# Varkalandar/raysnail

Hardware: AMD Instinct MI355X
Metric: Msamples/s (whole node) + ms/frame, RTIOW-13.1 scene 800x500x64spp (higher is better)
Workload: dtype f64; 1 GPU; rtow_13_1 balls_scene(seed 7)+light, 800x500, 64 spp, depth 8; width=800, height=500, spp=64, depth=8, split=rows, lanes=default, frames_in_flight=default, samples_per_frame=25600000

## Files before the change

raysnail_amd/csrc/rs_host.cpp:

```cpp
#include <hip/hip_runtime.h>

#include <algorithm>
#include <atomic>
#include <chrono>
#include <functional>
#include <cmath>
#include <cstdio>
#include <cstdlib>
#include <cstring>
#include <memory>
#include <new>
#include <stdexcept>
#include <string>
#include <vector>

#include "../../include/raysnail_hip.h"
#include "rs_host_util.h"
#include "rs_internal.h"
#include "rs_layout.h"
#include "rs_cull.h"

using namespace rs;

namespace {

thread_local std::string g_last_error;

struct Box3 {
    double lo[3], hi[3];
};
Box3 box_union(const Box3& a, const Box3& b) {
    Box3 r;
    for (int i = 0; i < 3; ++i) { r.lo[i] = std::fmin(a.lo[i], b.lo[i]); r.hi[i] = std::fmax(a.hi[i], b.hi[i]); }
    return r;
}
Box3 box_empty() {
    Box3 r;
    for (int i = 0; i < 3; ++i) { r.lo[i] = INFINITY; r.hi[i] = -INFINITY; }
    return r;
}

struct HObj {
    int32_t kind = 0;
    int32_t mat = RS_NO_MATERIAL;
    double p[18] = {0};
    int32_t a = -1, b = -1;
    int32_t ax[3] = {0, 0, 0};
    std::vector<rs_transform> tfs;
};

struct HPerlin {
    rs_perlin_desc d;
    std::vector<double> values;
// ... 78 lines not shown
};

struct CandKey {
    DCamera dc{};
    uint32_t width = 0, height = 0, row_begin = 0, row_step = 0, n_pix = 0;
    uint64_t gen = 0;
    bool valid = false;
    bool same(const CandKey& o) const {
        return valid && o.valid && std::memcmp(&dc, &o.dc, sizeof(DCamera)) == 0 && width == o.width && height == o.height &&
               row_begin == o.row_begin && row_step == o.row_step && n_pix == o.n_pix && gen == o.gen;
    }
};

struct Slot {
    hipStream_t lane[kMaxLanes] = {nullptr};
    hipEvent_t fork_ev = nullptr, join_ev[kMaxLanes] = {nullptr};
    hipEvent_t free_ev = nullptr, entry_ev = nullptr;
    bool free_rec = false;
    double* d_rad = nullptr; size_t rad_cap = 0;
    double* d_acc = nullptr; size_t acc_cap = 0;
    unsigned long long* d_cnt = nullptr;
    uint8_t* d_mask = nullptr; size_t mask_cap = 0;
    float* d_out = nullptr; size_t out_cap = 0;
    float* d_feat = nullptr; size_t feat_cap = 0;
    void* d_wf = nullptr; size_t wf_cap = 0; uint32_t wf_lanes = 0; size_t wf_bytes = 0;
    QEnt** d_qptrs[kMaxLanes] = {nullptr};
    QEnt* qptr[kMaxLanes][kWfsClasses] = {{nullptr}};
    WfState lane_ws[kMaxLanes]{};
    uint32_t* d_counts = nullptr; size_t counts_cap = 0;
    size_t counts_clean = 0;
    hipStream_t acc_stream = nullptr;
    std::vector<hipEvent_t> bev;
    uint32_t* h_hist = nullptr; size_t hist_cap = 0, hist_words = 0; uint64_t hist_sig = 0;
    hipEvent_t hist_ev = nullptr; bool hist_pending = false;
    uint4* d_cand = nullptr; size_t cand_cap = 0;
    CandKey cand_key{};

    void quiesce() {
        for (uint32_t l = 0; l < kMaxLanes; ++l)
            if (lane[l]) HIP_OK(hipStreamSynchronize(lane[l]));
        if (acc_stream) HIP_OK(hipStreamSynchronize(acc_stream));
        if (free_rec) HIP_OK(hipEventSynchronize(free_ev));
    }
    void release() {
        for (uint32_t l = 0; l < kMaxLanes; ++l)
            if (lane[l]) (void)hipStreamSynchronize(lane[l]);
        if (acc_stream) (void)hipStreamSynchronize(acc_stream);
        if (free_rec) (void)hipEventSynchronize(free_ev);
        for (void* p : {(void*)d_rad, (void*)d_acc, (void*)d_cnt, (void*)d_mask, (void*)d_out, (void*)d_feat, d_wf, (void*)d_counts,
                        (void*)d_cand})
            if (p) (void)hipFree(p);
        for (uint32_t l = 0; l < kMaxLanes; ++l) {
            if (lane[l]) (void)hipStreamDestroy(lane[l]);
            if (join_ev[l]) (void)hipEventDestroy(join_ev[l]);
        }
        for (hipEvent_t e : {fork_ev, free_ev, entry_ev})
            if (e) (void)hipEventDestroy(e);
        for (hipEvent_t e : bev) (void)hipEventDestroy(e);
        if (acc_stream) (void)hipStreamDestroy(acc_stream);
        if (hist_ev) (void)hipEventDestroy(hist_ev);
        if (h_hist) (void)hipHostFree(h_hist);
    }
};

struct Replica {
    int device = 0;
    hipStream_t stream = nullptr;
    DScene ds{};
    std::vector<void*> dev;
    Slot slots[kMaxSlots];
    uint32_t next_slot = 0;
    int n_cu = 0, ext_bpc = 0, shade_bpc = 0;
    uint64_t mem_total = 0;
    int32_t* d_ovf = nullptr; size_t ovf_cap = 0;
    DScene* d_ds = nullptr;
    DScene uploaded{};
    std::vector<uint32_t> hist;
    uint64_t hist_sig = 0;
    std::vector<hipStream_t> pad_streams;

    void quiesce() {
        for (Slot& sl : slots) sl.quiesce();
        if (stream) HIP_OK(hipStreamSynchronize(stream));
    }
    SceneRef ref() {
        if (std::memcmp(&uploaded, &ds, sizeof(DScene)) != 0) {
            quiesce();
            HIP_OK(hipMemcpy(d_ds, &ds, sizeof(DScene), hipMemcpyHostToDevice));
            uploaded = ds;
        }
        return SceneRef{&ds, d_ds};
    }

    ~Replica() {
        int prev = -1;
        const bool switched = hipGetDevice(&prev) == hipSuccess && prev != device && hipSetDevice(device) == hipSuccess;
        for (Slot& sl : slots) sl.release();
        if (stream) (void)hipStreamSynchronize(stream);
        for (hipStream_t st : pad_streams) (void)hipStreamDestroy(st);
        for (void* p : dev) (void)hipFree(p);
        for (void* p : {(void*)d_ovf, (void*)d_ds})
            if (p) (void)hipFree(p);
        if (stream) (void)hipStreamDestroy(stream);
        if (switched) (void)hipSetDevice(prev);
    }
};

struct rs_scene {
    std::vector<rs_material_desc> mdesc;
    std::vector<HPerlin> perlins;
    std::vector<HImage> images;
    std::vector<HObj> objs;
    std::vector<uint32_t> world, lights;
    float bg_lo[3] = {0.3f, 0.4f, 0.5f}, bg_hi[3] = {0.7f, 0.89f, 1.0f};
    bool committed = false;
    bool spheres_only = false;
    int scene_mode = kSmGeneric;
    bool ref_order = false;
    HostScene hs;
    std::vector<std::unique_ptr<Replica>> reps;
    uint64_t max_items_per_batch = 32ull << 20;
    uint64_t pool_paths = 256ull << 20;
    uint32_t inject_div = 1;
    uint32_t finish_after = 16;
    uint32_t wf_lanes = 2;
    uint32_t stream_lanes = 1;
    uint32_t frames_in_flight = 3;
    bool ext_split = false;
    bool shade_split = true;
    bool dump_iters = false;
    uint32_t passes_stream = 0;
    uint32_t class_mask = (1u << kWfsClasses) - 1;
    int tree_depth = 0;
    int tree_arity = 0;
    int stack_need = 0;
    uint64_t commit_gen = 0;
    size_t n_nodes = 0;
    size_t n_leaf_entries = 0;
    double time0 = 0.0, time1 = 0.0;

    uint32_t add(HObj o) {
        if (committed) throw Error(RS_E_STATE, "scene already committed");
        objs.push_back(std::move(o));
        return (uint32_t)(objs.size() - 1);
    }
    void check_mat(int32_t m) const {
        if (m != RS_NO_MATERIAL && (m < 0 || (size_t)m >= mdesc.size())) throw Error(RS_E_INVALID, "unknown material id");
    }
    void check_handle(uint32_t h) const {
        if (h >= objs.size()) throw Error(RS_E_INVALID, "unknown object handle");
    }

    Box3 bbox(uint32_t h) { return bbox_t(h, time0, time1); }
    Box3 bbox_t(uint32_t h, double time0, double time1) {
        const HObj& o = objs[h];
        Box3 r;
        switch (o.kind) {
        case PK_SPHERE: {
            const double* c = o.p; const double rad = o.p[3]; const double* v = o.p + 5;
            Box3 s, e;
            if (v[0] == 0.0 && v[1] == 0.0 && v[2] == 0.0) {
                for (int i = 0; i < 3; ++i) { s.lo[i] = c[i] - rad; s.hi[i] = c[i] + rad; }
                return s;
// ... 855 lines not shown
    std::vector<double> tf64;
    std::vector<int32_t> ti32;
    for (const HPerlin& hp : s->perlins) {
        DPerlin x;
        std::memset(&x, 0, sizeof(x));
        x.point_count = (int32_t)hp.d.point_count; x.vector = hp.d.vector; x.smooth = hp.d.smooth; x.type = hp.d.type;
        x.depth = (int32_t)hp.d.depth; x.scale = hp.d.scale;
        x.voff = (int32_t)tf64.size(); x.poff = (int32_t)ti32.size();
        tf64.insert(tf64.end(), hp.values.begin(), hp.values.end());
        ti32.insert(ti32.end(), hp.perms.begin(), hp.perms.end());
        dper.push_back(x);
    }
    std::vector<DImage> dimg;
    std::vector<uint8_t> tu8;
    for (const HImage& hi : s->images) {
        DImage x; x.w = hi.w; x.h = hi.h; x.off = tu8.size();
        tu8.insert(tu8.end(), hi.rgb.begin(), hi.rgb.end());
        dimg.push_back(x);
    }
    stage(s, d.perlins, dper);
    stage(s, d.tex_f64, tf64);
    stage(s, d.tex_i32, ti32);
    stage(s, d.images, dimg);
    stage(s, d.tex_u8, tu8);
    d.uv = 0;
    for (const DMaterial& m : mats) if (m.tex_kind == RS_TEX_IMAGE) d.uv = 1;
    stage(s, d.lights, lights);
    d.n_lights = (int32_t)lights.size();
    d.root = root;
    d.default_mat = default_mat;
    d.ref_order = s->ref_order ? 1 : 0;
    for (int i = 0; i < 3; ++i) { d.bg_lo[i] = s->bg_lo[i]; d.bg_hi[i] = s->bg_hi[i]; }
    d.bg_lo[3] = d.bg_hi[3] = 1.0f;
    build_limg(s);
}

void commit(rs_scene* s, const int* devices, int n) {
    if (s->committed) throw Error(RS_E_STATE, "scene already committed");
    if (n < 0 || (n > 1 && !devices)) throw Error(RS_E_INVALID, "bad device list");
    build(s);
    int current = 0;
    if (n == 1 && !devices) {
        HIP_OK(hipGetDevice(&current));
        devices = &current;
    }
    int count = 0;
    if (n > 0) HIP_OK(hipGetDeviceCount(&count));
    for (int i = 0; i < n; ++i)
        if (devices[i] < 0 || devices[i] >= count) throw Error(RS_E_INVALID, "device ordinal out of range");
    int prev = 0;
    if (n > 0) HIP_OK(hipGetDevice(&prev));
    try {
        for (int i = 0; i < n; ++i) upload_replica(s, devices[i]);
        for (int i = 0; i < n; ++i)
            for (int j = 0; j < n; ++j) {
                if (devices[i] == devices[j]) continue;
                int can = 0;
                if (hipDeviceCanAccessPeer(&can, devices[i], devices[j]) == hipSuccess && can) {
                    (void)hipSetDevice(devices[i]);
                    (void)hipDeviceEnablePeerAccess(devices[j], 0);
                    (void)hipGetLastError();
                }
            }
    } catch (...) {
        s->reps.clear();
        (void)hipSetDevice(prev);
// ... 399 lines not shown
void accumulate_last(const Pending& P, const double* rad, uint32_t planes, bool first, const FinalParams& fp, float* out) {
    const size_t nz = P.counted ? 0 : P.n_counts;
    HIP_OK(launch_accumulate(rad, P.L->d_acc, P.n_pix, planes, first, 1, fp, out, P.L->d_counts, (uint32_t)nz, P.stream));
    P.L->counts_clean = nz;
}

struct PoolNeed { uint64_t cap; uint32_t lanes; size_t rad; };
template <class Plan, class Alloc>
void fit_pool(const rs_scene* s, const Replica& R, Slot& L, uint32_t want, uint64_t floor, Plan plan, Alloc alloc) {
    uint64_t pool = pool_limit(s, R, want);
    PoolNeed need = plan(pool);
    const uint64_t pool_min = std::min<uint64_t>(need.cap, floor);
    if (need.cap > L.wf_cap || need.lanes > L.wf_lanes || need.rad > L.rad_cap) {
        const uint64_t fp = std::max(pool_min, pool_limit_free(s, R, L, want, need.rad * sizeof(double)));
        if (fp < pool) need = plan(pool = fp);
    }
    while (!alloc(need)) {
        if (pool <= pool_min) throw Error(RS_E_NOMEM, "device memory exhausted: no room for the frame's path pool");
        need = plan(pool = std::max<uint64_t>(pool_min, pool / 2));
    }
}

void enqueue_empty(const FrameConsts& c, Pending& P) {
    Slot& L = *P.L;
    HIP_OK(hipMemsetAsync(L.d_acc, 0, (size_t)3 * P.n_pix * sizeof(double), L.lane[0]));
    join_to_end(L, P.stream);
    HIP_OK(launch_finalize(L.d_acc, c.d_out, c.fp, P.stream));
}

struct GridHist {
    uint64_t sig = 0;
    std::vector<size_t> hoff;
    size_t hwords = 0;
    bool hint = false;
};
GridHist hist_begin(Replica& R, Slot& L, const FrameSched& f, uint32_t n_pix, uint32_t N, uint32_t D, uint32_t n_frames) {
    GridHist h;
    h.sig = splitmix64_h(((uint64_t)n_pix << 32) ^ N) ^ splitmix64_h(((uint64_t)D << 40) ^ ((uint64_t)f.lanes << 32) ^ n_frames);
    for (const LaneSched& ln : f.lane) {
        h.sig = splitmix64_h(h.sig ^ ln.Q ^ (ln.T << 40) ^ (ln.total << 1) ^ (uint64_t)ln.finish);
        h.hoff.push_back(h.hwords);
        h.hwords += 2 * ln.T;
    }
    for (Slot& o : R.slots) {
        if (!o.hist_pending) continue;
        const hipError_t q = hipEventQuery(o.hist_ev);
        if (q == hipSuccess) {
            o.hist_pending = false;
            R.hist.assign(o.h_hist, o.h_hist + o.hist_words);
            R.hist_sig = o.hist_sig;
        } else {
            (void)hipGetLastError();
            if (q != hipErrorNotReady) HIP_OK(q);
        }
    }
#ifndef RS_NO_GRID_HINT
    h.hint = R.hist_sig == h.sig && R.hist.size() == h.hwords;
#endif
    if (L.hist_cap < h.hwords) {
        if (L.h_hist) { HIP_OK(hipEventSynchronize(L.hist_ev)); HIP_OK(hipHostFree(L.h_hist)); L.h_hist = nullptr; }
        HIP_OK(hipHostMalloc((void**)&L.h_hist, h.hwords * sizeof(uint32_t)));
        L.hist_cap = h.hwords;
        L.hist_pending = false;
    }
    if (!L.hist_ev) HIP_OK(hipEventCreateWithFlags(&L.hist_ev, hipEventDisableTiming));
    return h;
}
uint64_t hist_grid(const GridHist& h, const Replica& R, uint32_t l, uint64_t t, int word, uint64_t n_max, uint64_t more = 0) {
    if (!h.hint) return n_max;
    const uint64_t est = R.hist[h.hoff[l] + 2 * t + word];
    return std::min<uint64_t>(n_max, est + est / 4 + 64ull * kBlock + more);
}
void hist_end(const GridHist& h, Slot& L, const FrameSched& f, hipStream_t S) {
    for (uint32_t l = 0; l < f.lanes; ++l)
        HIP_OK(hipMemcpy2DAsync(L.h_hist + h.hoff[l], 2 * sizeof(uint32_t), L.d_counts + f.lane[l].cnt_off,
                                kWfsStride * sizeof(uint32_t), 2 * sizeof(uint32_t), f.lane[l].T,
                                hipMemcpyDeviceToHost, S));
    HIP_OK(hipEventRecord(L.hist_ev, S));
    L.hist_pending = true;
    L.hist_sig = h.sig;
    L.hist_words = h.hwords;
}

bool cam_cand_scene(const rs_scene* s, const DScene& d) {
    return cam_cand(s->scene_mode, kExtCamera) && d.moving == 0 && d.lsphs && d.root4 >= 0 && !d.ref_order &&
           s->objs.size() <= kCandMaxEntries && s->stack_need <= kCandStack;
}
const uint4* cam_cand_records(const rs_scene* s, const FrameConsts& c, Slot& L, hipStream_t L0) {
    const PathParams& pp = c.pp;
    if (!cam_cand_scene(s, *c.ds.host) || pp.n_pix_local == 0 || pp.n_pix_local > (0xFFFFFFFFu >> 4)) return nullptr;
    if (!cand_camera(c.dc.origin, c.dc.lb, c.dc.hf, c.dc.vf, c.dc.hu, c.dc.vu, c.dc.aperture, pp.width, pp.height).ok)
        return nullptr;
    CandKey key;
    key.dc = c.dc;
    key.width = pp.width; key.height = pp.height; key.row_begin = pp.row_begin; key.row_step = pp.row_step;
    key.n_pix = pp.n_pix_local;
    key.gen = s->commit_gen;
    key.valid = true;
    if (L.cand_key.same(key)) return L.d_cand;
    L.cand_key.valid = false;
    if (!try_ensure(L, L.d_cand, L.cand_cap, std::max<size_t>(pp.n_pix_local, (size_t)pp.width * pp.height))) return nullptr;
    HIP_OK(launch_cam_cand_build(c.ds, c.dc, pp, L.d_cand, L0));
    L.cand_key = key;
    return L.d_cand;
}

struct StreamFrame {
    const rs_scene* s; const FrameConsts& c; Pending& P; Slot& L;
    const uint4* cand = nullptr;
    FrameSched f;
    GridHist h;
    bool split, split_shade;
    std::vector<uint64_t> window;
    hipEvent_t done_ev(uint32_t k) const { return L.bev[2 * (size_t)k]; }
    hipEvent_t acc_ev(uint32_t k) const { return L.bev[2 * (size_t)k + 1]; }
    void iteration(uint32_t l, uint64_t t);
    void accumulate(uint32_t k);
};

void StreamFrame::iteration(uint32_t l, uint64_t t) {
    const bool timed = P.timed;
    const uint32_t D = P.depth;
    const int sm = s->scene_mode;
    const LaneSched& ln = f.lane[l];
    const hipStream_t cs = L.lane[l];
    WfState WS = L.lane_ws[l];
    WS.tagw = tag_in_ray(c.ds, c.dc);
    WS.counts = L.d_counts + ln.cnt_off;
    QEnt** qd = L.d_qptrs[l];
    const uint32_t n_new = ln.n_new(t);
    P.inj[l][t] = n_new;
    InjParams I = inj_params(f, ln, t);
    I.cand = cand;
    if (n_new) {
        const uint64_t m = t * ln.Q / f.B;
        for (uint64_t mm = m; mm <= m + 1 && mm < ln.batch.size(); ++mm) {
            const uint32_t kk = ln.batch[mm];
            if (ln.first_it(mm) == t && kk >= f.ring) HIP_OK(hipStreamWaitEvent(cs, acc_ev(kk - f.ring), 0));
        }
    }
    if (ln.finish && t + 1 == ln.T) {
        const uint32_t b = (uint32_t)std::min<uint64_t>(c.wide, (window[l] + kBlock - 1) / kBlock);
        if (timed) HIP_OK(hipEventRecord(P.kev[2 * P.ki], cs));
        HIP_OK(launch_wfs_finish(c.ds, WS, (uint32_t)t, D, L.d_rad, std::max<uint32_t>(1, b), sm, cs));
        if (timed) HIP_OK(hipEventRecord(P.kev[2 * P.ki + 1], cs));
        ++P.ki;
        ++P.path_launches;
        window[l] = 0;
        return;
    }
    auto extend = [&](int part, uint64_t n_max) {
        if (part == kExtCarried) n_max = hist_grid(h, *P.R, l, t, 0, n_max);
        const uint32_t b = (uint32_t)std::min<uint64_t>(c.ext_cap, (n_max + kBlock - 1) / kBlock);
        if (!b) return;
        HIP_OK(launch_wfs_extend(c.ds, c.dc, c.pp, WS, qd, (uint32_t)t, I, L.d_rad, b, part, sm, cs,
                                 timed ? P.kev[2 * P.ki] : nullptr, timed ? P.kev[2 * P.ki + 1] : nullptr));
        ++P.ki;
        ++P.path_launches;
    };
    if (split) {
// ... 32 lines not shown
                                 nullptr, 0, L.acc_stream));
        HIP_OK(hipEventRecord(acc_ev(k), L.acc_stream));
        return;
    }
    join(L.join_ev[0], L.acc_stream, S);
    HIP_OK(hipStreamWaitEvent(S, done_ev(k), 0));
    join_lanes(L, f.lanes, S);
    join(L.fork_ev, L.lane[0], S);
    hist_end(h, L, f, S);
    accumulate_last(P, rk, planes, kl == 0, c.fp, out);
}

void enqueue_streaming(const rs_scene* s, const rs_render_settings* st, const FrameConsts& c, Pending& P) {
    Slot& L = *P.L;
    const hipStream_t L0 = L.lane[0];
    const uint32_t n_pix = P.n_pix, N = P.N, D = P.depth, n_frames = P.n_frames;
    StreamFrame F{s, c, P, L};
    FrameSched& f = F.f;
    const uint32_t want = c.ext_spill ? 1u : std::min<uint32_t>(kMaxLanes, s->stream_lanes);
    fit_pool(s, *P.R, L, want, (uint64_t)65536 * std::max<uint32_t>(D, 1),
             [&](uint64_t pool) {
                 f = make_sched(s, n_pix, N, D, want, pool, n_frames);
                 return PoolNeed{f.cap, f.lanes, (size_t)3 * f.ring * f.B};
             },
             [&](const PoolNeed& need) {
                 if (carve_wf(L, need.cap, need.lanes) && try_ensure(L, L.d_rad, L.rad_cap, need.rad)) return true;
                 release_pool(L);
                 return false;
             });
    f.keys.resize(n_frames);
    for (uint32_t k = 0; k < n_frames; ++k)
        f.keys[k] = splitmix64_h(splitmix64_h(st->seed) ^ (uint64_t)(st->pass + k));
    prepare_counts(L, P.n_counts = f.n_counts, L0);
    F.h = hist_begin(*P.R, L, f, n_pix, N, D, n_frames);
    if (!L.acc_stream) HIP_OK(hipStreamCreateWithFlags(&L.acc_stream, hipStreamNonBlocking));
    F.cand = cam_cand_records(s, c, L, L0);
    fork_lanes(L, f.lanes);
    HIP_OK(hipStreamWaitEvent(L.acc_stream, L.fork_ev, 0));
    if (n_frames > 1) HIP_OK(hipStreamWaitEvent(L.acc_stream, c.outs_after, 0));
    while (L.bev.size() < 2 * (size_t)f.n_batches) {
        hipEvent_t e;
        HIP_OK(hipEventCreateWithFlags(&e, hipEventDisableTiming));
        L.bev.push_back(e);
    }
    F.split = ext_split(s->scene_mode) || s->ext_split || n_frames > 1;
    F.split_shade = s->shade_split && (uint64_t)n_pix * N >= kSplitShadeMin;
    size_t n_ext = 0;
    for (const LaneSched& ln : f.lane) n_ext += ln.T * (F.split ? 2 : 1);
    new_events(P.kev, P.timed ? 2 * n_ext : 0);
    new_events(P.ev, P.timed ? 2 : 0);
    if (P.timed) HIP_OK(hipEventRecord(P.ev[0], L0));
    P.lanes.assign(f.lane.begin(), f.lane.end());
    F.window.assign(f.lanes, 0);
    P.inj.resize(f.lanes);
    for (uint32_t l = 0; l < f.lanes; ++l) P.inj[l].assign(f.lane[l].T, 0u);
    walk(f, [&](uint32_t l, uint64_t t) { F.iteration(l, t); },
         [&](uint32_t l, uint32_t k) { HIP_OK(hipEventRecord(F.done_ev(k), L.lane[l])); },
         [&](uint32_t k) { F.accumulate(k); });
    if (P.timed) HIP_OK(hipEventRecord(P.ev[1], P.stream));
}
void count_streaming(const rs_scene* s, const Pending& P, rs_render_stats* stats) {
    uint64_t seg = 0, kbytes = 0;
    for (size_t l = 0; l < P.lanes.size(); ++l)
        for (uint64_t t = 0; t < P.lanes[l].T; ++t) {
            const uint32_t* q = &P.qc[P.lanes[l].cnt_off + t * kWfsStride];
            uint64_t live_new = 0, shaded = 0, fused = 0;
            for (uint32_t k = 0; k < kStatLines; ++k) live_new += q[cix(kCntStat0 + (int)k)];
// ... 796 lines not shown

int rs_abi_version(void) { return RS_ABI_VERSION; }
const char* rs_last_error(void) { return g_last_error.c_str(); }
int rs_device_count(int* count) {
    return run([&] { if (!count) throw Error(RS_E_INVALID, "null"); HIP_OK(hipGetDeviceCount(count)); });
}
uint64_t rs_stream_key(uint64_t seed, uint32_t pass, uint64_t pixel, uint32_t sample) {
    return splitmix64_h(splitmix64_h(splitmix64_h(splitmix64_h(seed) ^ (uint64_t)pass) ^ pixel) ^ (uint64_t)sample);
}
double rs_medium_uniform(const uint32_t st[4], uint32_t handle) {
    const uint64_t key = splitmix64_h((((uint64_t)st[1] << 32) | st[0]) ^ splitmix64_h(((uint64_t)st[3] << 32) | st[2]));
    return (double)splitmix64_h(key ^ splitmix64_h(0x6d656469756d2121ULL + (uint64_t)handle)) * 0x1p-64;
}

int rs_scene_create(rs_scene** out) {
    return run([&] {
        if (!out) throw Error(RS_E_INVALID, "null");
        rs_scene* s = new rs_scene();
#ifdef RS_DEV_KNOBS
        auto knob = [](const char* name, unsigned long long& v) {
            if (const char* e = std::getenv(name)) { const unsigned long long x = std::strtoull(e, nullptr, 10); if (x) v = x; }
        };
        unsigned long long v;
        v = s->max_items_per_batch; knob("RS_MAX_BATCH_ITEMS", v); s->max_items_per_batch = v;
        v = s->pool_paths; knob("RS_POOL_PATHS", v); s->pool_paths = v;
        v = s->inject_div; knob("RS_INJECT_DIV", v); s->inject_div = (uint32_t)v;
        if (const char* e = std::getenv("RS_FINISH_AFTER")) s->finish_after = (uint32_t)std::strtoul(e, nullptr, 10);
        v = s->wf_lanes; knob("RS_LANES", v); s->wf_lanes = (uint32_t)std::min<unsigned long long>(v, kMaxLanes);
        v = s->stream_lanes; knob("RS_SLANES", v); s->stream_lanes = (uint32_t)std::min<unsigned long long>(v, kMaxLanes);
        v = s->frames_in_flight; knob("RS_FRAMES", v); s->frames_in_flight = (uint32_t)std::min<unsigned long long>(v, kMaxSlots);
        v = 0; knob("RS_EXT_SPLIT", v); s->ext_split = v != 0;
        v = 0; knob("RS_SHADE_MERGED", v); if (v) s->shade_split = false;
        v = 0; knob("RS_DUMP_ITERS", v); s->dump_iters = v != 0;
        v = 0; knob("RS_PASSES_STREAM", v); s->passes_stream = (uint32_t)v;
#endif
        *out = s;
    });
}
int rs_scene_destroy(rs_scene* s) {
    return run([&] { delete s; });
}
int rs_material(rs_scene* s, const rs_material_desc* d, int32_t* id) {
    return run([&] {
        S(s);
        if (!d || !id) throw Error(RS_E_INVALID, "null argument");
        if (s->committed) throw Error(RS_E_STATE, "scene already committed");
        if (d->kind < RS_MAT_LAMBERTIAN || d->kind > RS_MAT_BLINN_PHONG) throw Error(RS_E_INVALID, "unknown material kind");
        if (d->texture.kind < RS_TEX_SOLID || d->texture.kind > RS_TEX_IMAGE) throw Error(RS_E_INVALID, "unknown texture kind");
        if (d->texture.kind == RS_TEX_PERLIN && (d->texture.data < 0 || (size_t)d->texture.data >= s->perlins.size()))
            throw Error(RS_E_INVALID, "texture refers to an unknown rs_perlin id");
        if (d->texture.kind == RS_TEX_IMAGE && (d->texture.data < 0 || (size_t)d->texture.data >= s->images.size()))
            throw Error(RS_E_INVALID, "texture refers to an unknown rs_image id");
        if (d->kind == RS_MAT_MIXED) {
            if (d->mix_a < 0 || (size_t)d->mix_a >= s->mdesc.size() || d->mix_b < 0 || (size_t)d->mix_b >= s->mdesc.size())
                throw Error(RS_E_INVALID, "mixed material refers to unknown ids");
        }
        *id = (int32_t)s->mdesc.size();
        s->mdesc.push_back(*d);
    });
}
int rs_perlin(rs_scene* s, const rs_perlin_desc* d, int32_t* id) {
    return run([&] {
        S(s);
        if (!d || !id || !d->values || !d->perm_x || !d->perm_y || !d->perm_z) throw Error(RS_E_INVALID, "null argument");
        if (s->committed) throw Error(RS_E_STATE, "scene already committed");
        const uint32_t n = d->point_count;
// ... 542 lines not shown
```

raysnail_amd/csrc/rs_internal.h:

```cpp
#pragma once
#include <hip/hip_runtime.h>
#include <stdint.h>
#include "rs_layout.h"
#include "rs_cam_cand.h"
#include "rs_light_cand.h"

namespace rs {

constexpr int kBlock = 256;
constexpr int kStackMax = 24;
constexpr int kStackMin = 16;
constexpr uint32_t kLeafBatch = 8;
constexpr uint32_t kMaxLanes = 4;
constexpr uint32_t kMaxSlots = 4;
constexpr int kMaxFrames = 64;

enum SceneMode { kSmGeneric = 0, kSmSpheres = 1, kSmFlat = 2, kSmNest0 = 3, kSmNest2 = 4, kSmMarch = 5 };
constexpr bool generic_mode(int sm) { return sm == kSmGeneric || sm == kSmMarch; }
constexpr int march_of(int sm) { return sm == kSmMarch ? 1 : 0; }
constexpr int nest_of(int sm) { return sm == kSmNest0 ? 0 : sm == kSmNest2 ? 2 : generic_mode(sm) ? RS_MAX_NEST : 0; }
constexpr int rich_of(int sm) { return generic_mode(sm) ? 1 : 0; }
constexpr bool streaming_mode(int sm) { return sm == kSmSpheres || sm == kSmNest0 || sm == kSmNest2; }
constexpr int stack_lds(int sm) { return generic_mode(sm) ? kStackMax : kStackMin; }
static_assert(4u * ((uint32_t)stack_lds(kSmNest0) * kBlock * 4u + kLimgMax) <= 160u * 1024u, "LDS image budget");
// ... 17 lines not shown
struct PathParams {
    uint64_t n_items;
    uint32_t n_pix_local;
    uint32_t width, height;
    uint32_t row_begin, row_step;
    uint32_t sqrt_spp;
    uint32_t s0;
    uint32_t depth;
    uint64_t key_base;
    const uint8_t* mask;
};

struct alignas(32) D4 { double x, y, z, w; };
struct alignas(16) QEnt {
    uint32_t i;
    int32_t bp;
    double t;
};

struct WfSet {
    D4* ray_o;
    D4* ray_d;
    D4* thr;
    uint2* tag;
};
struct WfState {
    WfSet set[2];
    double2* hit;
    uint32_t* counts;
    uint32_t* fetch;
    uint32_t* heads;
    uint32_t cap;
    uint32_t tagw;
};

struct InjParams {
    uint32_t n_new;
    uint32_t jb0;
    uint32_t nb0;
    uint32_t nb1;
    uint64_t g0, g1;
    uint32_t rad0, rad1;
    uint64_t key0, key1;
    const uint4* cand;
};

struct FinalParams {
    uint32_t n_pix_local, width, row_begin, row_step;
    uint32_t n_samples;
    int32_t gamma;
    const uint8_t* mask;
};

hipError_t launch_probe_sample(const SceneRef& s, const DCamera& c, const PathParams& p, int sm, uint32_t x, uint32_t y,
                               uint32_t s0, uint32_t n, double* out, hipStream_t st);
hipError_t launch_probe_shade(const SceneRef& s, const double* rows, uint32_t n, uint64_t key_base, double* out, int sm,
                              hipStream_t st);
hipError_t launch_probe_camera(const DCamera& c, const PathParams& p, const uint32_t* xys, uint32_t n, int centres,
                               double* out, int sm, hipStream_t st);
hipError_t launch_path_mega(const SceneRef& s, const DCamera& c, const PathParams& p, int sm, double* rad,
                            unsigned long long* seg_counters, uint32_t max_blocks, hipStream_t st);
hipError_t launch_wf_gen(const DCamera& c, const PathParams& p, const WfState& w, uint64_t item0, uint32_t n, double* rad,
                         hipStream_t st);
hipError_t launch_wf_extend(const SceneRef& s, const WfState& w, uint32_t bounce, uint32_t blocks, int sm, hipStream_t st);
hipError_t launch_wf_shade(const SceneRef& s, const WfState& w, uint32_t bounce, uint32_t depth, uint64_t n_items, double* rad,
                           uint32_t blocks, int sm, hipStream_t st);
// ... 74 lines not shown
```

raysnail_amd/csrc/rs_kernels.hip:

```cpp
#include <cstdlib>
#include <type_traits>

#include <hip/hip_ext.h>

#include "rs_device.h"
#include "rs_internal.h"
#include "rs_gen_perm.h"
#include "rs_cull.h"

#define RS_PASTE_(a, b) a##b
#define RS_PASTE(a, b) RS_PASTE_(a, b)
#if !defined(RS_TU)
#define RS_TU_COMMON 1
#define RS_TU_MODES 1
#define RS_TU_SUFFIX
#elif RS_TU < 0
#define RS_TU_COMMON 1
#define RS_TU_MODES 0
#define RS_TU_SUFFIX _c
#elif RS_TU == 6
#define RS_TU_COMMON 0
#define RS_TU_MODES 0
#define RS_TU_SUFFIX _6
#elif RS_TU == 7
// ... 705 lines not shown
        return false;
    }
    double light_multi = 1.0, pdf_val;
    Ray nr;
    nr.time = ray.time;
    if (rng.gen() < 0.5) {
        if (light_ray) *light_ray = 1;
        pdf_val = 0.3183098861837907;
        const uint32_t li = rng.next_u32() % (uint32_t)S.n_lights;
        V3 rv;
        if (SM == kSmSpheres) rv = Obj<0, 0>::sphere_random(S.spheres[S.prims[S.lights[li]].idx], h.p, rng);
        else if (SM == kSmFlat) rv = Obj<0, 0>::random(S, S.lights[li], h.p, rng);
        else rv = obj_random<SM>(S, S.lights[li], h.p, rng);
        V3 dl = unit(rv);
        if (M0.phong_factor > 0.0) light_multi += phong_highlight(-dl, ray.d, h.n, M0.phong_exponent, M0.phong_factor);
        nr.o = ray_at(ray, h.t1 - 0.0002);
        nr.d = dl;
    } else {
        V3 sd = (KIND == RS_MAT_LAMBERTIAN) ? onb_local(pdf.n, random_cosine_direction(rng))
                                            : pdf_generate<rich_of(SM)>(pdf, rng);
        pdf_val = pdf_value<rich_of(SM)>(pdf, sd);
        nr.o = h.p;
        nr.d = sd;
    }
    if (pdf_val <= 0.0 || pdf_val != pdf_val) pdf_val = 1e-5;
    const double mult = pdf_value<rich_of(SM)>(pdf, nr.d) / pdf_val;
    T = v3(((double)c[0] * (light_multi * T.x)) * mult, ((double)c[1] * (light_multi * T.y)) * mult,
           ((double)c[2] * (light_multi * T.z)) * mult);
    ray = nr;
    return true;
}

__device__ __forceinline__ V3 close_path(V3 L, V3 T) { return L + T * 0.0; }

template <int R>
__device__ __forceinline__ V3 emission(const DScene& S, const DMaterial& M0, const Hit& h) {
    float c[3];
    tex_color<R>(S, M0, h, c);
    return v3((double)c[0] * M0.multiplier, (double)c[1] * M0.multiplier, (double)c[2] * M0.multiplier);
}

template <int SM, int KIND = -1>
__device__ bool shade_step(const DScene& S, bool hit_ok, const Hit& h, Ray& ray, V3& T, V3& L, Rng& rng) {
    if (!hit_ok) {
        V3 bg = background(S, ray);
        L = L + v3(T.x * bg.x, T.y * bg.y, T.z * bg.z);
        return false;
    }
    const int mi = h.mat >= 0 ? h.mat : S.default_mat;
    const DMaterial& M0 = S.mats[mi];
    if (M0.kind == RS_MAT_DIFFUSE_LIGHT) {
        V3 e = emission<rich_of(SM)>(S, M0, h);
        L = L + v3(T.x * e.x, T.y * e.y, T.z * e.z);
        return false;
    }
    if constexpr (KIND == RS_MAT_LAMBERTIAN) {
        if (shade_surface<RS_MAT_LAMBERTIAN, SM>(S, h, M0, M0, ray, T, rng)) return true;
        L = close_path(L, T);
        return false;
    }
    int ms = mi;
    for (int k = 0; k < 16 && S.mats[ms].kind == RS_MAT_MIXED; ++k) {
        const DMaterial& X = S.mats[ms];
        ms = ((double)rng.next_u32() < 4294967295.0 * X.mix_p) ? X.mix_a : X.mix_b;
    }
    if (shade_surface<-1, SM>(S, h, M0, S.mats[ms], ray, T, rng)) return true;
// ... 601 lines not shown
        }
#ifdef RS_TRAV_STATS
        {
            const int c = gen ? 0 : j < nf ? 1 : 2;
            const unsigned long long lm = __ballot(live);
            trav_stats_flush(live, lm ? __shfl(c, __ffsll((long long)lm) - 1, 64) : 0);
        }
#endif
        uint32_t* const cs[kClasses] = {&cnt[cix(1)], &cnt[cix(2)], &cnt[cix(3)], &cnt[cix(4)], &cnt[cix(5)]};
        const uint32_t slot = block_slot<kClasses>(cls, cs, gen && live,
                                                   PART == kExtCarried ? nullptr : &cnt[cix(kCntStat0 + (int)(blockIdx.x % kStatLines))]);
        if (cls >= 0) {
            QEnt q;
            q.i = i; q.bp = qbp; q.t = qt;
            queues[cls][slot] = q;
        }
        if constexpr (kFuse) {
            bool alive = false;
            int light_ray = 0;
            V3 T = v3(1.0, 1.0, 1.0);
            if (fcls >= 0) {
                if (W.tagw) r.time = 0.0;
                r.key = 0;
                Hit h;
                const DPrim Pr = S.prims[qbp];
                sphere_rec_at(S.spheres[Pr.idx], Pr.mat, r, qt, h);
                const int mi = h.mat >= 0 ? h.mat : S.default_mat;
                const DMaterial& M0 = S.mats[mi];
                bool cont;
                if (fcls == 0) cont = shade_surface<RS_MAT_LAMBERTIAN, SM>(S, h, M0, M0, r, T, rng, &light_ray);
                else if (fcls == 1) cont = shade_surface<RS_MAT_METAL, SM>(S, h, M0, M0, r, T, rng, &light_ray);
                else cont = shade_surface<RS_MAT_DIELECTRIC, SM>(S, h, M0, M0, r, T, rng, &light_ray);
                alive = cont && (1u < P.depth);
                if (!alive) {
                    const V3 L = close_path(v3(0.0, 0.0, 0.0), T);
                    put_rad(rad, item, L.x, L.y, L.z);
                }
            }
            uint32_t* cnt_next = cnt + kWfsStride;
            uint32_t* const gc[2] = {&cnt_next[cix(kCntBack)], &cnt_next[cix(kCntFront)]};
            const uint32_t fslot = block_slot<2>(alive ? light_ray : -1, gc, fcls >= 0,
                                                 &cnt[cix(kCntStat0 + (int)(blockIdx.x % kStatLines)) + 1]);
            if (alive) {
                const uint32_t p = light_ray ? fslot : W.cap - 1u - fslot;
                store_path(W.set[(it + 1) & 1], p, r, T, rng, item, 1u, W.tagw);
            }
        }
    }
}

template <int SM, bool LOBJ>
__global__ __launch_bounds__(kBlock, 2) void k_wfs_finish(const DScene* __restrict__ Sp, WfState W, uint32_t it, uint32_t depth,
                                                      double* __restrict__ rad) {
    DScene Sv;
    if constexpr (LOBJ) lds_scene(Sp, Sv);
    const DScene& S = LOBJ ? Sv : *Sp;
    __shared__ int stk_all[stack_lds(SM) * kBlock];
    const StkT<true, stack_lds(SM)> stk = make_stk<true, stack_lds(SM)>(S, stk_all);
    uint32_t* cnt = W.counts + (size_t)it * kWfsStride;
    const uint32_t nf = cnt[cix(kCntFront)];
    const uint32_t n = nf + cnt[cix(kCntBack)];
    if (blockIdx.x == 0 && threadIdx.x == 0) cnt[0] = n;
    const WfSet& cur = W.set[it & 1];
    uint32_t extra = 0;
    for (uint32_t base = blockIdx.x * kBlock; base < n; base += gridDim.x * kBlock) {
        const uint32_t j = base + threadIdx.x;
        if (j >= n) continue;
        const uint32_t i = j < nf ? j : W.cap - 1u - (j - nf);
        Ray r;
        V3 T;
        Rng rng;
        uint2 tg;
        load_path(cur, i, r, T, rng, W.tagw, tg);
        V3 L = v3(0.0, 0.0, 0.0);
        bool open = true;
        for (uint32_t lvl = tg.y; lvl < depth; ++lvl) {
            if (lvl != tg.y) ++extra;
            Hit h;
            double bend;
            const int bp = traverse<SM, StkT<true, stack_lds(SM)>, LOBJ>(S, r, 0.0001, bend, stk);
            const bool ok = finish_hit<SM>(S, bp, r, 0.0001, bend, h);
            if (!shade_step<SM>(S, ok, h, r, T, L, rng)) { open = false; break; }
        }
        if (open) L = close_path(L, T);
        put_rad(rad, tg.x, L.x, L.y, L.z);
    }
    unsigned long long e = extra;
#pragma unroll
    for (int off = 32; off > 0; off >>= 1) e += __shfl_xor(e, off, 64);
    if ((threadIdx.x & 63) == 0 && e) atomicAdd(&cnt[cix(kCntStat0 + (int)(blockIdx.x % kStatLines))], (uint32_t)e);
}

template <int KIND, int SM>
__device__ __forceinline__ void wfs_shade_batch(const DScene& S, const WfState& W, const QEnt* __restrict__ queue,
                                                uint32_t n, uint32_t base, uint32_t it, uint32_t* cnt_next, uint32_t depth,
                                                double* __restrict__ rad) {
    const WfSet& cur = W.set[it & 1];
    const WfSet& nxt = W.set[(it + 1) & 1];
    const uint32_t j = base + threadIdx.x;
    bool alive = false;
    int light_ray = 0;
    Ray r;
    V3 T;
    Rng rng;
    uint32_t item = 0, lvl = 0;
    if (j < n) {
        const QEnt q = queue[j];
        const uint32_t i = q.i;
        uint2 tg;
        load_path(cur, i, r, T, rng, W.tagw, tg);
        item = tg.x;
        lvl = tg.y;
        const int bp = q.bp;
        Hit h;
        if constexpr (SM == kSmSpheres) {
            const DPrim P = S.prims[bp];
            sphere_rec_at(S.spheres[P.idx], P.mat, r, q.t, h);
        } else {
            finish_hit<SM, (KIND >= 0)>(S, bp, r, 0.0001, q.t, h);
        }
        const int mi = h.mat >= 0 ? h.mat : S.default_mat;
        const DMaterial& M0 = S.mats[mi];
        bool cont;
        if (KIND >= 0) {
            cont = shade_surface<KIND, SM>(S, h, M0, M0, r, T, rng, &light_ray);
        } else if (M0.kind == RS_MAT_DIFFUSE_LIGHT) {
            const V3 e = emission<0>(S, M0, h);
            const V3 L = v3(0.0, 0.0, 0.0) + v3(T.x * e.x, T.y * e.y, T.z * e.z);
            put_rad(rad, item, L.x, L.y, L.z);
            cont = false;
            item = ~0u;
        } else {
            int ms = mi;
            for (int k = 0; k < 16 && S.mats[ms].kind == RS_MAT_MIXED; ++k) {
                const DMaterial& X = S.mats[ms];
                ms = ((double)rng.next_u32() < 4294967295.0 * X.mix_p) ? X.mix_a : X.mix_b;
            }
            cont = shade_surface<-1, SM>(S, h, M0, S.mats[ms], r, T, rng, &light_ray);
        }
        alive = cont && (lvl + 1 < depth);
        if (!alive && item != ~0u) {
            const V3 L = close_path(v3(0.0, 0.0, 0.0), T);
            put_rad(rad, item, L.x, L.y, L.z);
        }
    }
    uint32_t* const gc[2] = {&cnt_next[cix(kCntBack)], &cnt_next[cix(kCntFront)]};
    const uint32_t slot = block_slot<2>(alive ? light_ray : -1, gc);
    if (alive) {
        const uint32_t p = light_ray ? slot : W.cap - 1u - slot;
        store_path(nxt, p, r, T, rng, item, lvl + 1u, W.tagw);
    }
}

template <int SM, bool G4, bool LOBJ, int PS>
#ifndef RS_LEAN_WAVES
#define RS_LEAN_WAVES 5
#endif
#define RS_SHADE_WAVES(SM, G4, LOBJ, PS) (SM == kSmSpheres ? (PS == 1 ? RS_LEAN_WAVES : 4) : PS == 1 ? 4 : (SM == kSmNest2 && G4 && !LOBJ) ? 1 : 3)
__global__ __launch_bounds__(kBlock, RS_SHADE_WAVES(SM, G4, LOBJ, PS)) void k_wfs_shade_all(const DScene* __restrict__ Sp, WfState W,
                                                                                   QEnt* const* __restrict__ queues,
                                                                                   uint32_t class_mask, uint32_t it,
                                                                                   uint32_t depth,
                                                                                   double* __restrict__ rad) {
    DScene Sv;
    if constexpr (LOBJ) lds_scene(Sp, Sv);
    const DScene& S = LOBJ ? Sv : *Sp;
    const uint32_t* cnt = W.counts + (size_t)it * kWfsStride;
    uint32_t* cnt_next = W.counts + (size_t)(it + 1) * kWfsStride;
    constexpr int NC = G4 ? 5 : 4;
    constexpr uint32_t kPart = PS == 0 ? 0x1fu : PS == 1 ? 0x0bu : 0x14u;
    uint32_t n[NC], first[NC + 1];
    first[0] = 0;
#pragma unroll
// ... 1156 lines not shown
```

raysnail_amd/csrc/rs_layout.h:

```cpp
#pragma once
#include <stdint.h>
#include "rs_light_cand.h"

#define RS_MAX_NEST 4

namespace rs {

enum PrimKind : int32_t {
    PK_SPHERE = 0,
    PK_RECT = 1,
    PK_BOX = 2,
    PK_QUADRIC = 3,
    PK_TRIANGLE = 4,
    PK_AND = 5,
    PK_SUB = 6,
    PK_XFORM = 7,
    PK_MEDIUM = 8,
    PK_RAYMARCH = 9,
};

struct DPrim {
    int32_t kind;
    int32_t idx;
    int32_t mat;
// ... 128 lines not shown
    const DBox* boxes;
    const DQuadric* quadrics;
    const DTri* tris;
    const DCsg* csgs;
    const DXform* xforms;
    const DMat34* tf_fwd;
    const DMat34* tf_inv;
    const DMaterial* mats;
    const DMedium* media;
    const DPerlin* perlins;
    const DImage* images;
    const double* tex_f64;
    const int32_t* tex_i32;
    const uint8_t* tex_u8;
    const int32_t* lights;
    int32_t* stk_ovf;
    const void* limg;
    uint32_t limg_bytes;
    uint32_t limg_off[LT_COUNT];
    int32_t n_lights;
    int32_t root;
    int32_t default_mat;
    int32_t ref_order;
    int32_t root4;
    int32_t uv;
    int32_t has_media;
    int32_t stack_need;
    int32_t moving;
    int32_t ltop;
    int32_t lamb_only;
    float bg_lo[4], bg_hi[4];
    LightGrid lgrid;
    const uint32_t* lcand;
};

#ifndef RS_LTOP
#define RS_LTOP 85
#endif
constexpr int kLTop = RS_LTOP;


struct DCamera {
    double origin[3], lb[3], hf[3], vf[3], hu[3], vu[3];
    double aperture, shutter;
};

}
```

Baseline: 5219 Msamples/s.

## Terminate sphere-scene paths early once throughput becomes exactly zero

```diff
diff --git a/raysnail_amd/csrc/rs_dead_gate.h b/raysnail_amd/csrc/rs_dead_gate.h
--- /dev/null
+++ b/raysnail_amd/csrc/rs_dead_gate.h
@@ -0,0 +1,78 @@
+#pragma once
+#include <math.h>
+#include <stdint.h>
+
+#include "rs_layout.h"
+
+namespace rs {
+
+constexpr double kDeadBig = 0x1p100;
+constexpr double kDeadReach = 0x1p20;
+constexpr double kDeadMargin = 0x1p-20;
+
+inline bool dead_num(double x) { return fabs(x) <= kDeadBig; }
+
+struct DeadGateIn {
+    bool spheres_mode = false;
+    bool moving = false;
+    const DMaterial* mats = nullptr; uint32_t n_mats = 0;
+    const DSphere* spheres = nullptr; uint32_t n_spheres = 0;
+    const uint32_t* lights = nullptr; uint32_t n_lights = 0;
+    const float* bg_lo = nullptr; const float* bg_hi = nullptr;
+};
+
+inline double dead_gate_reach(const DeadGateIn& g) {
+    if (!g.spheres_mode || g.moving) return 0.0;
+    for (int k = 0; k < 3; ++k)
+        if (!dead_num((double)g.bg_lo[k]) || !dead_num((double)g.bg_hi[k])) return 0.0;
+    for (uint32_t i = 0; i < g.n_mats; ++i) {
+        const DMaterial& m = g.mats[i];
+        for (int k = 0; k < 3; ++k)
+            if (!dead_num((double)m.even[k]) || !dead_num((double)m.odd[k])) return 0.0;
+        if (!dead_num(m.multiplier) || !dead_num(m.enter_refractive) || !dead_num(m.outer_refractive) ||
+            !dead_num(m.mix_p) || !dead_num(m.phong_factor) || !dead_num(m.exponent))
+            return 0.0;
+        if (!(m.exponent >= 0.0) || m.phong_factor > 0.0) return 0.0;
+    }
+    if (g.n_spheres == 0) return 0.0;
+    double rho = INFINITY, M = 0.0;
+    for (uint32_t i = 0; i < g.n_spheres; ++i) {
+        const DSphere& s = g.spheres[i];
+        const double r = fabs(s.r);
+        if (!dead_num(r) || !(r > 0.0)) return 0.0;
+        if (s.v[0] != 0.0 || s.v[1] != 0.0 || s.v[2] != 0.0) return 0.0;
+        if (r < rho) rho = r;
+        for (int k = 0; k < 3; ++k) {
+            if (!dead_num(s.c[k])) return 0.0;
+            if (fabs(s.c[k]) + r > M) M = fabs(s.c[k]) + r;
+        }
+    }
+    if (!(rho >= 1.0 / kDeadBig) || !(M <= kDeadReach * rho)) return 0.0;
+    for (uint32_t a = 0; a < g.n_lights; ++a) {
+        if (g.lights[a] >= g.n_spheres) return 0.0;
+        const DSphere& l = g.spheres[g.lights[a]];
+        const double rl = fabs(l.r);
+        for (uint32_t i = 0; i < g.n_spheres; ++i) {
+            if (i == g.lights[a]) continue;
+            const DSphere& s = g.spheres[i];
+            const double rs = fabs(s.r);
+            const double dx = s.c[0] - l.c[0], dy = s.c[1] - l.c[1], dz = s.c[2] - l.c[2];
+            const double d = sqrt(dx * dx + dy * dy + dz * dz);
+            const bool apart = d > (rs + rl) * (1.0 + kDeadMargin);
+            const bool inside = (d + rl) * (1.0 + kDeadMargin) < rs;
+            if (!apart && !inside) return 0.0;
+        }
+    }
+    return M;
+}
+
+inline bool dead_gate(const DeadGateIn& g) { return dead_gate_reach(g) > 0.0; }
+
+inline bool dead_gate_camera(double reach, const double origin[3]) {
+    if (!(reach > 0.0)) return false;
+    for (int k = 0; k < 3; ++k)
+        if (!(fabs(origin[k]) <= 2.0 * reach)) return false;
+    return true;
+}
+
+}
diff --git a/raysnail_amd/csrc/rs_host.cpp b/raysnail_amd/csrc/rs_host.cpp
--- a/raysnail_amd/csrc/rs_host.cpp
+++ b/raysnail_amd/csrc/rs_host.cpp
@@ -19,6 +19,7 @@
 #include "rs_internal.h"
 #include "rs_layout.h"
 #include "rs_cull.h"
+#include "rs_dead_gate.h"
 
 using namespace rs;
 
@@ -163,6 +164,7 @@
     hipStream_t acc_stream = nullptr;
     std::vector<hipEvent_t> bev;
     uint32_t* h_hist = nullptr; size_t hist_cap = 0, hist_words = 0; uint64_t hist_sig = 0;
+    int hist_bank = 0;
     hipEvent_t hist_ev = nullptr; bool hist_pending = false;
     uint4* d_cand = nullptr; size_t cand_cap = 0;
     CandKey cand_key{};
@@ -206,8 +208,8 @@
     int32_t* d_ovf = nullptr; size_t ovf_cap = 0;
     DScene* d_ds = nullptr;
     DScene uploaded{};
-    std::vector<uint32_t> hist;
-    uint64_t hist_sig = 0;
+    std::vector<uint32_t> hist[2];
+    uint64_t hist_sig[2] = {0, 0};
     std::vector<hipStream_t> pad_streams;
 
     void quiesce() {
@@ -260,6 +262,7 @@
     bool ext_split = false;
     bool shade_split = true;
     bool dump_iters = false;
+    bool dead_in_stats = false;
     uint32_t passes_stream = 0;
     uint32_t class_mask = (1u << kWfsClasses) - 1;
     int tree_depth = 0;
@@ -1181,6 +1184,20 @@
     d.ref_order = s->ref_order ? 1 : 0;
     for (int i = 0; i < 3; ++i) { d.bg_lo[i] = s->bg_lo[i]; d.bg_hi[i] = s->bg_hi[i]; }
     d.bg_lo[3] = d.bg_hi[3] = 1.0f;
+    {
+        DeadGateIn g;
+        g.spheres_mode = s->scene_mode == kSmSpheres;
+        g.moving = d.moving != 0;
+        g.mats = mats.data(); g.n_mats = (uint32_t)mats.size();
+        g.spheres = spheres.data(); g.n_spheres = (uint32_t)spheres.size();
+        std::vector<uint32_t> lsph;
+        for (int32_t h : lights)
+            if (prims[h].kind == PK_SPHERE) lsph.push_back((uint32_t)prims[h].idx);
+            else g.spheres_mode = false;
+        g.lights = lsph.data(); g.n_lights = (uint32_t)lsph.size();
+        g.bg_lo = d.bg_lo; g.bg_hi = d.bg_hi;
+        d.dead_reach = dead_gate_reach(g);
+    }
     build_limg(s);
 }
 
@@ -1646,10 +1663,13 @@
     uint64_t sig = 0;
     std::vector<size_t> hoff;
     size_t hwords = 0;
+    int bank = 0;
     bool hint = false;
 };
-GridHist hist_begin(Replica& R, Slot& L, const FrameSched& f, uint32_t n_pix, uint32_t N, uint32_t D, uint32_t n_frames) {
+GridHist hist_begin(Replica& R, Slot& L, const FrameSched& f, uint32_t n_pix, uint32_t N, uint32_t D, uint32_t n_frames,
+                    bool end_dead) {
     GridHist h;
+    h.bank = end_dead ? 1 : 0;
     h.sig = splitmix64_h(((uint64_t)n_pix << 32) ^ N) ^ splitmix64_h(((uint64_t)D << 40) ^ ((uint64_t)f.lanes << 32) ^ n_frames);
     for (const LaneSched& ln : f.lane) {
         h.sig = splitmix64_h(h.sig ^ ln.Q ^ (ln.T << 40) ^ (ln.total << 1) ^ (uint64_t)ln.finish);
@@ -1661,15 +1681,15 @@
         const hipError_t q = hipEventQuery(o.hist_ev);
         if (q == hipSuccess) {
             o.hist_pending = false;
-            R.hist.assign(o.h_hist, o.h_hist + o.hist_words);
-            R.hist_sig = o.hist_sig;
+            R.hist[o.hist_bank].assign(o.h_hist, o.h_hist + o.hist_words);
+            R.hist_sig[o.hist_bank] = o.hist_sig;
         } else {
             (void)hipGetLastError();
             if (q != hipErrorNotReady) HIP_OK(q);
         }
     }
 #ifndef RS_NO_GRID_HINT
-    h.hint = R.hist_sig == h.sig && R.hist.size() == h.hwords;
+    h.hint = R.hist_sig[h.bank] == h.sig && R.hist[h.bank].size() == h.hwords;
 #endif
     if (L.hist_cap < h.hwords) {
         if (L.h_hist) { HIP_OK(hipEventSynchronize(L.hist_ev)); HIP_OK(hipHostFree(L.h_hist)); L.h_hist = nullptr; }
@@ -1682,7 +1702,7 @@
 }
 uint64_t hist_grid(const GridHist& h, const Replica& R, uint32_t l, uint64_t t, int word, uint64_t n_max, uint64_t more = 0) {
     if (!h.hint) return n_max;
-    const uint64_t est = R.hist[h.hoff[l] + 2 * t + word];
+    const uint64_t est = R.hist[h.bank][h.hoff[l] + 2 * t + word];
     return std::min<uint64_t>(n_max, est + est / 4 + 64ull * kBlock + more);
 }
 void hist_end(const GridHist& h, Slot& L, const FrameSched& f, hipStream_t S) {
@@ -1693,6 +1713,7 @@
     HIP_OK(hipEventRecord(L.hist_ev, S));
     L.hist_pending = true;
     L.hist_sig = h.sig;
+    L.hist_bank = h.bank;
     L.hist_words = h.hwords;
 }
 
@@ -1725,6 +1746,7 @@
     FrameSched f;
     GridHist h;
     bool split, split_shade;
+    bool end_dead = false;
     std::vector<uint64_t> window;
     hipEvent_t done_ev(uint32_t k) const { return L.bev[2 * (size_t)k]; }
     hipEvent_t acc_ev(uint32_t k) const { return L.bev[2 * (size_t)k + 1]; }
@@ -1740,6 +1762,7 @@
     const hipStream_t cs = L.lane[l];
     WfState WS = L.lane_ws[l];
     WS.tagw = tag_in_ray(c.ds, c.dc);
+    WS.end_dead = end_dead ? 1u : 0u;
     WS.counts = L.d_counts + ln.cnt_off;
     QEnt** qd = L.d_qptrs[l];
     const uint32_t n_new = ln.n_new(t);
@@ -1838,7 +1861,8 @@
     for (uint32_t k = 0; k < n_frames; ++k)
         f.keys[k] = splitmix64_h(splitmix64_h(st->seed) ^ (uint64_t)(st->pass + k));
     prepare_counts(L, P.n_counts = f.n_counts, L0);
-    F.h = hist_begin(*P.R, L, f, n_pix, N, D, n_frames);
+    F.end_dead = (!P.counted || s->dead_in_stats) && dead_gate_camera(c.ds.host->dead_reach, c.dc.origin);
+    F.h = hist_begin(*P.R, L, f, n_pix, N, D, n_frames, F.end_dead);
     if (!L.acc_stream) HIP_OK(hipStreamCreateWithFlags(&L.acc_stream, hipStreamNonBlocking));
     F.cand = cam_cand_records(s, c, L, L0);
     fork_lanes(L, f.lanes);
@@ -2701,6 +2725,7 @@
         v = 0; knob("RS_EXT_SPLIT", v); s->ext_split = v != 0;
         v = 0; knob("RS_SHADE_MERGED", v); if (v) s->shade_split = false;
         v = 0; knob("RS_DUMP_ITERS", v); s->dump_iters = v != 0;
+        v = 0; knob("RS_DEAD_IN_STATS", v); s->dead_in_stats = v != 0;
         v = 0; knob("RS_PASSES_STREAM", v); s->passes_stream = (uint32_t)v;
 #endif
         *out = s;
diff --git a/raysnail_amd/csrc/rs_internal.h b/raysnail_amd/csrc/rs_internal.h
--- a/raysnail_amd/csrc/rs_internal.h
+++ b/raysnail_amd/csrc/rs_internal.h
@@ -73,6 +73,7 @@
     uint32_t* heads;
     uint32_t cap;
     uint32_t tagw;
+    uint32_t end_dead;
 };
 
 struct InjParams {
diff --git a/raysnail_amd/csrc/rs_kernels.hip b/raysnail_amd/csrc/rs_kernels.hip
--- a/raysnail_amd/csrc/rs_kernels.hip
+++ b/raysnail_amd/csrc/rs_kernels.hip
@@ -761,6 +761,12 @@
 }
 
 __device__ __forceinline__ V3 close_path(V3 L, V3 T) { return L + T * 0.0; }
+
+template <int SM>
+__device__ __forceinline__ bool dead_path(const WfState& W, V3 T) {
+    if constexpr (SM != kSmSpheres) return false;
+    return W.end_dead && T.x == 0.0 && T.y == 0.0 && T.z == 0.0;
+}
 
 template <int R>
 __device__ __forceinline__ V3 emission(const DScene& S, const DMaterial& M0, const Hit& h) {
@@ -1428,6 +1434,7 @@
                 else if (fcls == 1) cont = shade_surface<RS_MAT_METAL, SM>(S, h, M0, M0, r, T, rng, &light_ray);
                 else cont = shade_surface<RS_MAT_DIELECTRIC, SM>(S, h, M0, M0, r, T, rng, &light_ray);
                 alive = cont && (1u < P.depth);
+                if (dead_path<SM>(W, T)) alive = false;
                 if (!alive) {
                     const V3 L = close_path(v3(0.0, 0.0, 0.0), T);
                     put_rad(rad, item, L.x, L.y, L.z);
@@ -1477,6 +1484,7 @@
             const int bp = traverse<SM, StkT<true, stack_lds(SM)>, LOBJ>(S, r, 0.0001, bend, stk);
             const bool ok = finish_hit<SM>(S, bp, r, 0.0001, bend, h);
             if (!shade_step<SM>(S, ok, h, r, T, L, rng)) { open = false; break; }
+            if (dead_path<SM>(W, T)) break;
         }
         if (open) L = close_path(L, T);
         put_rad(rad, tg.x, L.x, L.y, L.z);
@@ -1535,6 +1543,7 @@
             cont = shade_surface<-1, SM>(S, h, M0, S.mats[ms], r, T, rng, &light_ray);
         }
         alive = cont && (lvl + 1 < depth);
+        if (dead_path<SM>(W, T)) alive = false;
         if (!alive && item != ~0u) {
             const V3 L = close_path(v3(0.0, 0.0, 0.0), T);
             put_rad(rad, item, L.x, L.y, L.z);
diff --git a/raysnail_amd/csrc/rs_layout.h b/raysnail_amd/csrc/rs_layout.h
--- a/raysnail_amd/csrc/rs_layout.h
+++ b/raysnail_amd/csrc/rs_layout.h
@@ -184,6 +184,7 @@
     float bg_lo[4], bg_hi[4];
     LightGrid lgrid;
     const uint32_t* lcand;
+    double dead_reach;
 };
 
 #ifndef RS_LTOP
```

New measurement: 5994 Msamples/s (median of 6 runs). 14.8% higher.
